# pxl-th/SLAM.jl

Hardware: AMD Instinct MI355X
Metric: frames/sec KITTI-05 stereo @1k kpts; local-BA ms/iter for 50-KF window (higher is better)
Workload: dtype f64

## Files before the change

### slam.jl_amd/csrc/common.hpp

```cpp
#pragma once
#include <hip/hip_runtime.h>
#include <cstdint>
#include <cstdio>
#include <cstring>
#include <string>
#include <vector>
#include <mutex>
#include "../../include/slamhip.h"

#define SLAM_MAX_LEVELS 8

struct slam_ctx {
    int device = 0;
    hipStream_t stream = nullptr;
    int cus = 0;
    int dev_cus = 0;
    bool arch_ok = false;
    bool xwg_ok = false;
    int pool_class = 99;
    std::string err;
    void *scratch = nullptr; size_t scratch_bytes = 0;
    void *scratch2 = nullptr; size_t scratch2_bytes = 0;
    void *pinned = nullptr; size_t pinned_bytes = 0;
    hipEvent_t wait_event = nullptr;
// ... 5 lines not shown
    std::vector<hipEvent_t> prof_pool;
    std::vector<std::string> prof_names;
    std::vector<double> prof_ms;
    std::vector<long long> prof_cnt;
};

extern "C" hipStream_t ctx_aux_stream(slam_ctx *c);
extern "C" void ctx_probe_device(slam_ctx *c);

struct ProfScope {
    slam_ctx *c; int idx;
    ProfScope(slam_ctx *ctx, const char *name);
    ~ProfScope();
};

struct LevelView {
    double *L, *Iy, *Ix, *Iyy, *Ixx, *Iyx;
    int H, W, P;
};
struct PyrView {
    LevelView lv[SLAM_MAX_LEVELS];
    int levels;
};

struct slam_pyr {
    int device = 0;
    int levels = 0;
    int H[SLAM_MAX_LEVELS], W[SLAM_MAX_LEVELS];
    int P[SLAM_MAX_LEVELS];
    int64_t off[SLAM_MAX_LEVELS + 1];
    struct Alloc { double *base = nullptr; double *ck = nullptr; double *tot = nullptr; const void **srctab = nullptr; double *xc = nullptr; int *xf = nullptr; int xseg = 0; double *rck = nullptr; int refs = 0; std::mutex graph_mu; };
    Alloc *alloc = nullptr;
    size_t zstride = 0;
    int batch_index = 0, batch_size = 1;
    bool tol_planes = false;
    bool target_only = false;
    double *planes = nullptr;
    double *tmp = nullptr;
    double *ck = nullptr;
    double *norm = nullptr;
    double norm_sigma = -1.0;
    struct Graph { int mode; double sigma; int S; size_t ckmin; int src_kind; hipGraphExec_t exec; };
    std::vector<Graph> graphs;
    bool graph_failed = false;
    PyrView view;
    double *plane(int p, int l) const { return planes + (int64_t)p * off[levels] + off[l]; }
};

struct slam_kpset {
    int device = 0, S = 0, cap = 0;
    char *base = nullptr;
    double *yx = nullptr;
    double *oyx = nullptr;
    double *syx = nullptr;
    double *xyz = nullptr;
    double *kyx = nullptr;
    uint8_t *haskf = nullptr;
    double *fyx = nullptr;
    int *fkf = nullptr;
    int *kfcount = nullptr;
    int64_t *id = nullptr;
// ... 61 lines not shown
```

### slam.jl_amd/csrc/lk.hip

```cpp
#include "common.hpp"
#include "geom_device.hpp"
#include <vector>
#include <cmath>
#include <cstdlib>

struct LKArgs {
    PyrView prev, cur;
    const double *pts, *disp0;
    int n, pyramid_levels, window, iterations;
    double eig_thr, eps, max_distance;
    double *out;
    uint8_t *status;
};

#ifdef LK_TRACE
__device__ unsigned long long g_lk_ticks[8];
#define LKT_BEGIN unsigned long long _t0 = wall_clock64()
#define LKT(k) do { const unsigned long long _t1 = wall_clock64(); if ((threadIdx.x & 63) == 0) atomicAdd(&g_lk_ticks[k], _t1 - _t0); _t0 = _t1; } while (0)
extern "C" int slam_debug_lk_ticks(unsigned long long *out)
{
    unsigned long long z[8] = {};
    if (hipMemcpyFromSymbol(out, HIP_SYMBOL(g_lk_ticks), sizeof z) != hipSuccess) return -1;
    return hipMemcpyToSymbol(HIP_SYMBOL(g_lk_ticks), z, sizeof z) == hipSuccess ? 0 : -1;
}
#else
#define LKT_BEGIN
#define LKT(k)
#endif

#define LK_OCC __attribute__((amdgpu_waves_per_eu(LK_MAXE == 9 ? 2 : 3, LK_MAXE == 9 ? 2 : 3)))
#define LK_PM 4
struct Offs { int up, down, left, right; };

__device__ __forceinline__ Offs get_offsets(int p0, int p1, double n0, double n1, int window, int H, int W)
{
    Offs o;
    const double q0 = (double)p0, q1 = (double)p1, w = (double)window;
    o.up = (int)floor(fmin(w, fmin(q0, n0) - 1));
    o.down = (int)floor(fmin(w, (double)H - fmax(q0, n0)));
    o.left = (int)floor(fmin(w, fmin(q1, n1) - 1));
    o.right = (int)floor(fmin(w, (double)W - fmax(q1, n1)));
    return o;
}

__device__ __forceinline__ double boxdiff(const double *I, int H, int y1, int y2, int x1, int x2)
{
// ... 84 lines not shown
    if (iy < 1) iy = 1;
    if (ix < 1) ix = 1;
    const double fy = r - iy, fx = c - ix;
    const double *p = img + (size_t)(iy - 1) + (size_t)(ix - 1) * P;
    const int dy = H > 1 ? 1 : 0; const size_t dx = W > 1 ? (size_t)P : 0;
    const double r0 = (1 - fx) * p[0] + fx * p[dx];
    const double r1 = (1 - fx) * p[dy] + fx * p[dy + dx];
    return (1 - fy) * r0 + fy * r1;
}

__device__ __forceinline__ bool lies_in(int H, int W, double a, double b)
{
    return 1.0 <= a && a <= (double)H && 1.0 <= b && b <= (double)W;
}

template <int LK_MAXE> struct Tmpl {
    double t0[LK_MAXE], t1[LK_MAXE], t2[LK_MAXE];
    int pq[LK_MAXE];
    int ne, kmax;
};
struct __attribute__((packed, aligned(8))) D2 { double a, b; };

template <int LK_MAXE, bool TOL>
__device__ __forceinline__ void load_template(Tmpl<LK_MAXE> &T, const LevelView &first, int p0, int p1, Offs o)
{
    const int lane = threadIdx.x & 63, pitch = first.P;
    const int P = o.up + o.down + 1, Q = o.left + o.right + 1, NE = P * Q;
    T.ne = NE; T.kmax = (NE + 63) >> 6;
    int pe, qe, sp, sq;
    if (P == 19) { pe = lane % 19; qe = lane / 19; sp = 64 % 19; sq = 64 / 19; }
    else if (P == 13) { pe = lane % 13; qe = lane / 13; sp = 64 % 13; sq = 64 / 13; }
    else if (P == 23) { pe = lane % 23; qe = lane / 23; sp = 64 % 23; sq = 64 / 23; }
    else { pe = lane % P; qe = lane / P; sp = 64 % P; sq = 64 / P; }
#pragma unroll
    for (int k = 0; k < LK_MAXE; k++) {
        const int e = lane + 64 * k;
        const bool in = e < NE;
        const int p = in ? pe : 0, q = in ? qe : 0;
        pe += sp; qe += sq;
        if (pe >= P) { pe -= P; qe++; }
        const size_t a = (size_t)(p0 - o.up + p - 1) + (size_t)(p1 - o.left + q - 1) * pitch;
        double v0 = 0.0, v1 = 0.0, v2 = 0.0;
        if (in) { v0 = first.L[a]; v1 = first.Iy[a]; v2 = first.Ix[a]; }
        T.t0[k] = in ? v0 : 0.0; T.t1[k] = in ? v1 : 0.0; T.t2[k] = in ? v2 : 0.0;
        T.pq[k] = TOL ? p + q * (2 * (LK_MAXE == 3 ? 6 : LK_MAXE == 6 ? 9 : 11) + 2 + 2 * LK_PM) : (p | (q << 16));
    }
}

template <int LK_MAXE> struct PatchGeom {
    static constexpr int WMAX = LK_MAXE == 3 ? 6 : LK_MAXE == 6 ? 9 : 11;
    static constexpr int PS = 2 * WMAX + 2 + 2 * LK_PM;
};
template <int PS>
__device__ __forceinline__ void stage_patch(double *patch, const double *img, int H, int W, int pitch, int cy, int cx, int &pry, int &prx)
{
    const int lane = threadIdx.x & 63;
    const int hy = H - PS, hx = W - PS;
    pry = cy < 0 ? 0 : (cy > hy ? (hy > 0 ? hy : 0) : cy);
    prx = cx < 0 ? 0 : (cx > hx ? (hx > 0 ? hx : 0) : cx);
    constexpr int CPC = PS / 2;
    constexpr int CPI = 64 / CPC;
    constexpr int NIT = (PS + CPI - 1) / CPI;
    const int ch = lane % CPC, c = lane / CPC;
    const double *src = img + (size_t)pry + (size_t)prx * pitch + (2 * ch + (size_t)c * pitch);
    const bool rows_ok = pry + 2 * ch < H;
#pragma unroll
    for (int i = 0; i < NIT; i++) {
        if (c < CPI && i * CPI + c < PS && rows_ok && prx + i * CPI + c < W)
            __builtin_amdgcn_global_load_lds((const __attribute__((address_space(1))) void *)(src + (size_t)(i * CPI) * pitch),
                                             (__attribute__((address_space(3))) void *)(patch + i * CPI * PS), 16, 0, 0);
    }
}

template <int LK_MAXE, bool TOL>
__device__ __forceinline__ bool lk_level(const LevelView &first, const LevelView &second, int level,
                         double pty, double ptx, double &dy, double &dx,
                         int window, int iterations, double eig_thr, double eps)
{
    const int lane = threadIdx.x & 63;
    const int H = first.H, W = first.W, pitch = first.P;
    const double iscale = __hiloint2double((1023 - (level - 1)) << 20, 0);
    const int p0 = (int)floor(pty * iscale), p1 = (int)floor(ptx * iscale);
    const double pf0 = (double)p0, pf1 = (double)p1;
    LKT_BEGIN;
    const bool cached = (2 * window + 1) * (2 * window + 1) <= 64 * LK_MAXE;
    Tmpl<LK_MAXE> T;
    constexpr int PS = PatchGeom<LK_MAXE>::PS;
    __shared__ __attribute__((aligned(16))) double lds_patch[PS * PS];
    int pry = 0, prx = 0;
    const int pmarg = (PS - (2 * window + 2)) >> 1;
    Offs o = {0, 0, 0, 0};
    double Gi[4];
    double c0 = 0.0, c1 = 0.0;
    for (int it = -1; it < iterations; it++) {
        double r0 = pf0, r1 = pf1;
        if (it >= 0) {
            const double f0 = dy + c0, f1 = dx + c1;
            r0 = pf0 + f0; r1 = pf1 + f1;
            if (!lies_in(H, W, r0, r1)) return false;
        }
        const Offs no = get_offsets(p0, p1, r0, r1, window, H, W);
        LKT(5);
        const double e0 = it < 0 ? pf0 + dy : r0, e1 = it < 0 ? pf1 + dx : r1;
        const double fr0 = floor(e0), fr1 = floor(e1);
        const int iy0 = (int)fr0, ix0 = (int)fr1;
        const bool fast = cached && iy0 - no.up >= 1 && iy0 + no.down <= H - 1 && ix0 - no.left >= 1 && ix0 + no.right <= W - 1;
        const int fy0 = iy0 - no.up - 1, fx0 = ix0 - no.left - 1;
        if (cached && (it < 0 || (fast && (fy0 < pry || iy0 + no.down > pry + PS - 1 || fx0 < prx || ix0 + no.right > prx + PS - 1))))
            stage_patch<PS>(lds_patch, second.L, H, W, pitch, iy0 - window - 1 - pmarg, ix0 - window - 1 - pmarg, pry, prx);
        if (it < 0 || no.up != o.up || no.down != o.down || no.left != o.left || no.right != o.right) {
            o = no;
            if (cached) load_template<LK_MAXE, TOL>(T, first, p0, p1, o);
            const double min_eig = spatial_gradient(first, p0, p1, o, Gi);
            LKT(1);
            if (min_eig < eig_thr) return false;
            LKT(2);
        }
        if (it < 0) continue;
        double ay = 0.0, ax = 0.0;
        if (fast) {
            asm volatile("s_waitcnt vmcnt(0)" ::: "memory");
            const double *pb = lds_patch + (fy0 - pry) + (fx0 - prx) * PS;
            constexpr int HS = (LK_MAXE + 1) / 2;
            if (TOL) {
                const double fy = r0 - fr0, fx = r1 - fr1;
#pragma unroll
                for (int h0 = 0; h0 < LK_MAXE; h0 += HS) {
                    D2 c0v[HS], c1v[HS];
#pragma unroll
                    for (int j = 0; j < HS; j++) {
                        const int k = h0 + j;
                        if (k < LK_MAXE && k < T.kmax) { const double *ptr = pb + T.pq[k]; c0v[j] = *(const D2 *)ptr; c1v[j] = *(const D2 *)(ptr + PS); }
                    }
#pragma unroll
                    for (int j = 0; j < HS; j++) {
                        const int k = h0 + j;
                        if (k < LK_MAXE && k < T.kmax) {
                            const double t0 = __builtin_fma(fx, c1v[j].a - c0v[j].a, c0v[j].a);
                            const double t1 = __builtin_fma(fx, c1v[j].b - c0v[j].b, c0v[j].b);
                            const double dI = T.t0[k] - __builtin_fma(fy, t1 - t0, t0);
                            ay = __builtin_fma(dI, T.t1[k], ay); ax = __builtin_fma(dI, T.t2[k], ax);
                        }
                    }
                }
            } else
#pragma unroll
            for (int h0 = 0; h0 < LK_MAXE; h0 += HS) {
                D2 c0v[HS], c1v[HS];
#pragma unroll
                for (int j = 0; j < HS; j++) {
                    const int k = h0 + j;
                    if (k < LK_MAXE && k < T.kmax) {
                        const double *ptr = pb + ((T.pq[k] & 0xffff) + (T.pq[k] >> 16) * PS);
                        c0v[j] = *(const D2 *)ptr; c1v[j] = *(const D2 *)(ptr + PS);
                    }
                }
#pragma unroll
                for (int j = 0; j < HS; j++) {
                    const int k = h0 + j;
                    if (k < LK_MAXE && k < T.kmax) {
                        const double dp = (double)((T.pq[k] & 0xffff) - o.up), dq = (double)((T.pq[k] >> 16) - o.left);
                        const double fy = (r0 + dp) - (fr0 + dp), fx = (r1 + dq) - (fr1 + dq);
                        const double t0 = (1 - fx) * c0v[j].a + fx * c1v[j].a;
                        const double t1 = (1 - fx) * c0v[j].b + fx * c1v[j].b;
                        const double dI = T.t0[k] - ((1 - fy) * t0 + fy * t1);
                        ay += dI * T.t1[k];
                        ax += dI * T.t2[k];
                    }
                }
            }
        } else {
            const int P = o.up + o.down + 1, Q = o.left + o.right + 1, NE = P * Q;
            for (int e = lane; e < NE; e += 64) {
                const int p = e % P, q = e / P;
                const double r = r0 + (double)(p - o.up), c = r1 + (double)(q - o.left);
                const size_t a = (size_t)(p0 - o.up + p - 1) + (size_t)(p1 - o.left + q - 1) * pitch;
                const double dI = first.L[a] - bilinear(second.L, H, W, pitch, r, c);
                ay += dI * first.Iy[a];
                ax += dI * first.Ix[a];
            }
        }
        LKT(3);
        wave_sum2(ay, ax);
        const double fl0 = TOL ? __builtin_fma(Gi[0], ay, Gi[2] * ax) : Gi[0] * ay + Gi[2] * ax, fl1 = TOL ? __builtin_fma(Gi[1], ay, Gi[3] * ax) : Gi[1] * ay + Gi[3] * ax;
        if (fabs(fl0) < eps && fabs(fl1) < eps) break;
        c0 += fl0; c1 += fl1;
        if (!lies_in(H, W, r0 + fl0, r1 + fl1)) return false;
        LKT(4);
    }
    dy += c0; dx += c1;
    if (level > 1) { dy *= 2.0; dx *= 2.0; }
    return true;
}

__device__ __forceinline__ LevelView shifted(const LevelView &v, size_t off)
{
    LevelView r = v;
    r.L += off; r.Iy += off; r.Ix += off; r.Iyy += off; r.Ixx += off; r.Iyx += off;
    return r;
}

template <int LK_MAXE, bool TOL = false>
__device__ __forceinline__ bool fb_point(const PyrView &prev, const PyrView &cur, double py, double px, double dy, double dx,
                                         int pyramid_levels, int window, int iterations, double eig_thr, double eps,
                                         double max_distance, double &ny, double &nx, size_t offP = 0, size_t offC = 0)
{
    double qy = py, qx = px, cy = dy, cx = dx;
    for (int k = 0; k <= pyramid_levels + 1; k++) {
        const bool back = k == pyramid_levels + 1;
        const int level = back ? 1 : pyramid_levels + 1 - k;
        if (back) {
            ny = py + cy; nx = px + cx;
            qy = ny; qx = nx;
// ... 333 lines not shown
```

### slam.jl_amd/csrc/pyramid.hip

```cpp
#include "common.hpp"
#include <cmath>
#include <cstdlib>
#include <mutex>
#include <tuple>
#include <utility>

#define LINE_THREADS 64

struct PlaneSet {
    double *p[4];
    const double *nrm[4];
    int coef[4];
    int fill0[4];
    const double *sq[4];
    int n;
    size_t zs;
};
#define PS_PICK(ps, f, pl) ((pl) == 0 ? (ps).f[0] : (pl) == 1 ? (ps).f[1] : (pl) == 2 ? (ps).f[2] : (ps).f[3])
__device__ __forceinline__ double *ps_plane(const PlaneSet &ps, int pl) { return PS_PICK(ps, p, pl) + (size_t)blockIdx.z * ps.zs; }
__device__ __forceinline__ const double *ps_nrm(const PlaneSet &ps, int pl) { return PS_PICK(ps, nrm, pl); }
__device__ __forceinline__ int ps_coef(const PlaneSet &ps, int pl) { return PS_PICK(ps, coef, pl); }
__device__ __forceinline__ bool ps_fill0(const PlaneSet &ps, int pl) { return PS_PICK(ps, fill0, pl) != 0; }
__device__ __forceinline__ const double *ps_sq(const PlaneSet &ps, int pl) { const double *q = PS_PICK(ps, sq, pl); return q ? q + (size_t)blockIdx.z * ps.zs : nullptr; }

// ... 106 lines not shown
    __device__ __forceinline__ bool valid() const { const int c = x0 + (int)(threadIdx.x & 63); return c >= slo && c <= shi; }
    __device__ __forceinline__ double ld_src(int i) const { return src[(size_t)i + (size_t)xown() * P]; }
    __device__ __forceinline__ double ld_dst(int i) const { return dst[(size_t)i + (size_t)xown() * P]; }
    __device__ __forceinline__ void st(int i, double v) const { if (valid()) dst[(size_t)i + (size_t)xown() * P] = v; }
    __device__ __forceinline__ void fence() const { __builtin_amdgcn_fence(__ATOMIC_RELEASE, "workgroup"); __builtin_amdgcn_fence(__ATOMIC_ACQUIRE, "workgroup"); }

    __device__ __forceinline__ void tile_load(const double *base, int rb, double t[16]) const
    {
        const int lane = threadIdx.x & 63, rp = lane & 7, cg = lane >> 3;
        const unsigned voff = (unsigned)(cg * P + 2 * rp);
#pragma unroll
        for (int r = 0; r < 8; r++) {
            const double *cb = base + ((size_t)(x0 + 8 * r) * P + rb);
            const double2 q = *(const double2 *)(cb + voff);
            t[2 * r] = q.x; t[2 * r + 1] = q.y;
        }
    }
    __device__ __forceinline__ void tile_store(int rb, const double t[16], int lo, int hi, bool partial) const
    {
        const int lane = threadIdx.x & 63, rp = lane & 7, cg = lane >> 3;
        const int row = rb + 2 * rp;
        const unsigned voff = (unsigned)(cg * P + 2 * rp);
#pragma unroll
        for (int r = 0; r < 8; r++) {
            const int col = x0 + 8 * r + cg;
            if (col >= slo && col <= shi) {
                double *q = dst + ((size_t)(x0 + 8 * r) * P + rb) + voff;
                if (!partial && nt) { const v2d v = {t[2 * r], t[2 * r + 1]}; __builtin_nontemporal_store(v, (v2d *)q); }
                else if (!partial) *(double2 *)q = make_double2(t[2 * r], t[2 * r + 1]);
                else {
// ... 360 lines not shown
    iir_rows_ck<false>(ps, H, W, P, cf, ck, rz);
}
__global__ __launch_bounds__(LINE_THREADS) void k_iir_rows_ck_odd(PlaneSet ps, int H, int W, int P, IIRPair cf, double *ck, RowResize rz)
{
    iir_rows_ck<true>(ps, H, W, P, cf, ck, rz);
}

__global__ __launch_bounds__(LINE_THREADS) void k_iir_cols_ck(PlaneSet ps, const double *src0, int H, int W, int P, IIRPair cf, double *ck)
{
    if (src0) src0 += (size_t)blockIdx.z * ps.zs;
    __shared__ __attribute__((aligned(16))) double tile[64 * COL_LS];
    const int pl = blockIdx.y, lane = threadIdx.x & 63;
    ColIO<2> io;
    const double *sqsrc = ps_sq(ps, pl);
    const bool sq = sqsrc != nullptr;
    io.dst = ps_plane(ps, pl); io.src = sq ? sqsrc : ((pl == 0 && src0) ? src0 : io.dst);
    io.H = H; io.W = W; io.P = P; io.x0 = blockIdx.x * LINE_THREADS; io.lds = tile; io.slo = 0; io.shi = W - 1; io.nt = true;
    const size_t nlines = (size_t)gridDim.z * gridDim.y * gridDim.x * LINE_THREADS;
    const size_t lineid = (((size_t)blockIdx.z * gridDim.y + pl) * gridDim.x + blockIdx.x) * LINE_THREADS + lane;
    const int n = H;
    const IIRCoef &k = ps_coef(ps, pl) == 0 ? cf.c[0] : cf.c[1];
    const bool fill0 = ps_fill0(ps, pl);
    const double a1 = k.a1, a2 = k.a2, a3 = k.a3, scale = k.scale;
    auto in = [&](double v) { return sq ? v * v : v; };
    const double x0 = in(io.ld_src(0));
    const double iminus = fill0 ? 0.0 : x0, iplus = fill0 ? 0.0 : in(io.ld_src(n - 1));
    const double uminus = iminus / k.inv1masum;
    const double o0 = ((x0 + a1 * uminus) + a2 * uminus) + a3 * uminus;
    const double o1 = ((in(io.ld_src(1)) + a1 * o0) + a2 * uminus) + a3 * uminus;
    const double o2 = ((in(io.ld_src(2)) + a1 * o1) + a2 * o0) + a3 * uminus;
    double w3 = o0, w2 = o1, w1 = o2;
    double raw[32], x[32];
    {
        const int NT = ((n - 1) >> 4) + 1;
        io.tile_load(io.src, 0, raw);
        for (int t = 0; t < NT; t++) {
            const int rb = t << 4;
            io.lds_put_tile(raw); io.template lds_get_col<+1>(x);
            if (sq) {
#pragma unroll
                for (int e = 0; e < 16; e++) x[e] = x[e] * x[e];
            }
            if (t + 1 < NT) io.tile_load(io.src, rb + 16, raw);
            if ((t & 1) == 0 && t >= 2) { double *c = ck + ((size_t)(t >> 1) * 3) * nlines + lineid; c[0] = w1; c[nlines] = w2; c[2 * nlines] = w3; }
            if (rb >= 3 && rb + 15 <= n - 1) {
#pragma unroll
                for (int e = 0; e < 16; e++) { const double tt = ((x[e] + a1 * w1) + a2 * w2) + a3 * w3; w3 = w2; w2 = w1; w1 = tt; }
            } else {
#pragma unroll
                for (int e = 0; e < 16; e++) { const int row = rb + e; if (row >= 3 && row <= n - 1) { const double tt = ((x[e] + a1 * w1) + a2 * w2) + a3 * w3; w3 = w2; w2 = w1; w1 = tt; } }
            }
        }
    }
    const double uplus = iplus / k.inv1masum, vplus = uplus / k.inv1mbsum;
    const double d0 = w1 - uplus, d1 = w2 - uplus, d2 = w3 - uplus;
    const double vr0 = ((k.M[0] * d0 + k.M[1] * d1) + k.M[2] * d2) + vplus;
    const double vr1 = ((k.M[3] * d0 + k.M[4] * d1) + k.M[5] * d2) + vplus;
    const double vr2 = ((k.M[6] * d0 + k.M[7] * d1) + k.M[8] * d2) + vplus;
    const double vA = vr0;
    const double vB = ((w2 + a1 * vA) + a2 * vr1) + a3 * vr2;
    const double vC = ((w3 + a1 * vB) + a2 * vA) + a3 * vr1;
    double v1 = vC, v2 = vB, v3 = vA;
    io.fence();
    const int NBk = ((n - 4) >> 5) + 1;
    const int ntile = P >> 4;
    auto load_block = [&](int b) {
        io.tile_load(io.src, b << 5, raw);
        if (2 * b + 1 < ntile) io.tile_load(io.src, (b << 5) + 16, raw + 16);
    };
    if (n - 4 >= 3) load_block(NBk - 1);
    io.st(n - 1, vA * scale); io.st(n - 2, vB * scale); io.st(n - 3, vC * scale);
    for (int b = NBk - 1; b >= 0 && n - 4 >= 3; b--) {
        const int rb = b << 5, lo = rb > 3 ? rb : 3, hi = rb + 31 < n - 4 ? rb + 31 : n - 4;
        const bool two = 2 * b + 1 < ntile;
        io.lds_put_tile(raw); io.template lds_get_col<+1>(x);
        if (two) { io.lds_put_tile(raw + 16); io.template lds_get_col<+1>(x + 16); }
        if (sq) {
#pragma unroll
            for (int e = 0; e < 32; e++) x[e] = x[e] * x[e];
        }
        if (b > 0) load_block(b - 1);
        double f1, f2, f3;
        if (b > 0) { const double *c = ck + ((size_t)b * 3) * nlines + lineid; f1 = c[0]; f2 = c[nlines]; f3 = c[2 * nlines]; }
// ... 16 lines not shown
            io.template lds_put_col<+1>(x + 16); io.lds_get_tile(u);
            io.tile_store(rb + 16, u, lo, hi, !(lo <= rb + 16 && hi >= rb + 31));
        }
    }
    {
        double tt = ((o2 + a1 * v1) + a2 * v2) + a3 * v3; v3 = v2; v2 = v1; v1 = tt; io.st(2, tt * scale);
        tt = ((o1 + a1 * v1) + a2 * v2) + a3 * v3; v3 = v2; v2 = v1; v1 = tt; io.st(1, tt * scale);
        tt = ((o0 + a1 * v1) + a2 * v2) + a3 * v3; io.st(0, tt * scale);
    }
}

#define CF4_COLS 62
struct ColsFusedArgs {
    const double *L;
    double *T;
    double *Iy, *Ix, *Qyy, *Qxx, *Qyx;
    int H, W, P; size_t zs;
    int src_kind; const void *const *srctab;
    double *tot; int tot_stride;
    int dec;
};

template <bool TOL>
__device__ __forceinline__ double iir3(double x, double a1, double w1, double a2, double w2, double a3, double w3)
{
    if (TOL) return __builtin_fma(a1, w1, __builtin_fma(a2, w2, __builtin_fma(a3, w3, x)));
    return ((x + a1 * w1) + a2 * w2) + a3 * w3;
}
template <bool TOL>
__device__ __forceinline__ void scharr_pair(double a, double b, double c, double &d, double &s)
{
// ... 89 lines not shown
__device__ __forceinline__ void cols_fused_wave(const ColsFusedArgs &A, const IIRCoef &k, double *ck, double *LB, double *IYB, double *IXB, double *QB, const double *lut)
{
    const int lane = threadIdx.x & 63, rp = lane & 7, cg = lane >> 3;
    const int H = A.H, W = A.W, P = A.P, n = H;
    const int own0 = CF4_COLS * (int)blockIdx.x;
    const int xl = own0 > 0 ? own0 - 1 : 0;
    const size_t z = (size_t)blockIdx.z * A.zs;
    const bool active = ROLE != 0 || A.T != nullptr;
    const int nroles = A.T != nullptr ? 4 : 3;
    double *stage = ROLE == 0 ? LB : ROLE == 1 ? IYB : ROLE == 2 ? IXB : QB;
    ColIO<2> io;
    io.src = A.L + z;
    io.dst = (ROLE == 0 ? A.T : ROLE == 1 ? A.Qyy : ROLE == 2 ? A.Qxx : A.Qyx) + z;
    io.H = H; io.W = W; io.P = P; io.x0 = xl; io.lds = stage;
    io.slo = own0; io.shi = own0 + CF4_COLS - 1 < W - 1 ? own0 + CF4_COLS - 1 : W - 1; io.nt = true;
    ColIO<2> iog = io;
    iog.dst = (ROLE == 1 ? A.Iy : A.Ix) + z;
    const int col = xl + lane;
    const bool edgeL = col == 0, edgeR = col == W - 1;
    const size_t nlines = (size_t)gridDim.z * nroles * gridDim.x * LINE_THREADS;
    const size_t lineid = (((size_t)blockIdx.z * nroles + (ROLE - (4 - nroles))) * gridDim.x + blockIdx.x) * LINE_THREADS + lane;
    const double a1 = k.a1, a2 = k.a2, a3 = k.a3, scale = k.scale;
    const int w = ROLE;
    const int skind = A.src_kind;
    typedef const __attribute__((address_space(1))) double *gsrc_f64;
    typedef const __attribute__((address_space(1))) unsigned char *gsrc_u8;
    typedef const __attribute__((address_space(3))) double *lds_f64;
    const void *simg = skind ? A.srctab[blockIdx.z] : nullptr;
    const gsrc_f64 simg_d = (gsrc_f64)simg; const gsrc_u8 simg_b = (gsrc_u8)simg; const lds_f64 lutl = (lds_f64)lut;
    auto src_at = [&](int row, int colx) -> double {
        return skind == 1 ? simg_d[(size_t)row + (size_t)colx * H] : lutl[simg_b[(size_t)row + (size_t)colx * H]];
    };
// ... 158 lines not shown
        lds_barrier();  
        if (active) read_inputs();
        if (ROLE == 0 && skind) {
            ColIO<2> iol = io; iol.dst = const_cast<double *>(A.L) + z;
            const int ghi = H - 1;
#pragma unroll
            for (int t = 0; t < 2; t++) {
                if (t == 0 || (two && rb + 16 <= ghi)) {
#pragma unroll
                    for (int r = 0; r < 8; r++) { const double2 q = *(const double2 *)(LB + (8 * r + cg) * CF4_LS + 2 + 16 * t + 2 * rp); u[2 * r] = q.x; u[2 * r + 1] = q.y; }
                    iol.tile_store(rb + 16 * t, u, rb + 16 * t, ghi, rb + 16 * t + 15 > ghi);
                }
            }
        }
        if (ROLE == 1 || ROLE == 2) {
            const double *blk = ROLE == 1 ? IYB : IXB;
            const int ghi = H - 1;
            get_tile(blk, 0, u); iog.tile_store(rb, u, rb, ghi, rb + 15 > ghi);
            if (two && rb + 16 <= ghi) { get_tile(blk, 1, u); iog.tile_store(rb + 16, u, rb + 16, ghi, rb + 31 > ghi); }
        }
        lds_barrier();
        double f1 = f1n, f2 = f2n, f3 = f3n;
        if (b > 0) { prefetch(b - 1); if (active) load_ck(b - 1); }
        if (!active || (lo > hi && !dec)) continue;
        if (lo > hi) {}
        else if (lo == rb && hi == rb + 31) {
#pragma unroll
            for (int e = 0; e < 32; e++) { const double tt = iir3<TOL>(x[e], a1, f1, a2, f2, a3, f3); f3 = f2; f2 = f1; f1 = tt; x[e] = tt; }
#pragma unroll
            for (int e = 31; e >= 0; e--) { const double tt = iir3<TOL>(x[e], a1, v1, a2, v2, a3, v3); v3 = v2; v2 = v1; v1 = tt;
                                            if (SFX) { x[e] = sfx; sfx = __builtin_fma(tt, scale, sfx); } else x[e] = tt * scale; }
        } else {
#pragma unroll
            for (int e = 0; e < 32; e++) { const int row = rb + e; if (row >= lo && row <= hi) { const double tt = iir3<TOL>(x[e], a1, f1, a2, f2, a3, f3); f3 = f2; f2 = f1; f1 = tt; x[e] = tt; } }
// ... 836 lines not shown
    ColTerm t; t.d = 0.0; t.s = 0.0;
    if (border == 0) xx = xx < 0 ? 0 : (xx >= W ? W - 1 : xx);
    else if (xx < 0 || xx >= W) return t;
    const double *c0 = L + (size_t)xx * P;
    double a, b, c;
    b = c0[y];
    if (border == 0) { a = c0[y > 0 ? y - 1 : 0]; c = c0[y + 1 < H ? y + 1 : H - 1]; }
    else { a = y > 0 ? c0[y - 1] : 0.0; c = y + 1 < H ? c0[y + 1] : 0.0; }
    t.d += a * dk[0]; t.d += b * dk[1]; t.d += c * dk[2];
    t.s += a * sk[0]; t.s += b * sk[1]; t.s += c * sk[2];
    return t;
}
template <int XC>
__global__ __launch_bounds__(64) void k_scharr_products(LevelView v, int border, size_t zs, int squares)
{
    { const size_t z = (size_t)blockIdx.z * zs; v.L += z; v.Iy += z; v.Ix += z; v.Iyy += z; v.Ixx += z; v.Iyx += z; }
    const int H = v.H, W = v.W, P = v.P;
    const int y = blockIdx.x * 64 + threadIdx.x;
    if (y >= H) return;
    const int xs = blockIdx.y * XC, xe = min(W, xs + XC);
    const double dk[3] = {-1.0 / 2, 0.0 / 2, 1.0 / 2}, sk[3] = {3.0 / 16, 10.0 / 16, 3.0 / 16};
    ColTerm t0 = scharr_col(v.L, H, W, P, y, xs - 1, border), t1 = scharr_col(v.L, H, W, P, y, xs, border);
    for (int x = xs; x < xe; x++) {
        const ColTerm t2 = scharr_col(v.L, H, W, P, y, x + 1, border);
        double iy = 0.0, ix = 0.0;
        iy += t0.d * sk[0]; iy += t1.d * sk[1]; iy += t2.d * sk[2];
        ix += t0.s * dk[0]; ix += t1.s * dk[1]; ix += t2.s * dk[2];
        const size_t i = (size_t)y + (size_t)x * P;
        v.Iy[i] = iy; v.Ix[i] = ix;
        if (squares) { v.Iyy[i] = iy * iy; v.Ixx[i] = ix * ix; }
        v.Iyx[i] = iy * ix;
        t0 = t1; t1 = t2;
    }
}

__global__ __launch_bounds__(256) void k_resize(double *dst, int Hd, int Wd, int Pd, const double *src, int Hs, int Ws, int Ps, size_t zs)
{
    dst += (size_t)blockIdx.z * zs; src += (size_t)blockIdx.z * zs;
    const size_t i = (size_t)blockIdx.x * 256 + threadIdx.x;
    if (i >= (size_t)Hd * Wd) return;
    const int y = (int)(i % Hd) + 1, x = (int)(i / Hd) + 1;
    const double sy = (double)Hs / (double)Hd, sx = (double)Ws / (double)Wd;
    const double oy = 1 - 0.5 - sy * (1 - 0.5), ox = 1 - 0.5 - sx * (1 - 0.5);
    double r = sy * y + oy, c = sx * x + ox;
// ... 19 lines not shown
}

#define BATCH_MAX 128
struct ImgPtrs { const double *p[BATCH_MAX]; };
__global__ __launch_bounds__(256) void k_gather_images(ImgPtrs src, double *dst, int H, int W, int P, size_t zs)
{
    const size_t i = (size_t)blockIdx.x * 256 + threadIdx.x;
    if (i < (size_t)H * W) dst[(size_t)blockIdx.z * zs + i % H + (i / H) * P] = src.p[blockIdx.z][i];
}
struct ImgPtrsU8 { const unsigned char *p[BATCH_MAX]; };
__global__ __launch_bounds__(256) void k_gather_images_u8(ImgPtrsU8 src, double *dst, int H, int W, int P, size_t zs)
{
    const size_t i = (size_t)blockIdx.x * 256 + threadIdx.x;
    if (i < (size_t)H * W) dst[(size_t)blockIdx.z * zs + i % H + (i / H) * P] = (double)src.p[blockIdx.z][i] / 255.0;
}
__global__ __launch_bounds__(256) void k_unpitch(double *dst, const double *src, int H, int W, int P)
{
    const size_t i = (size_t)blockIdx.x * 256 + threadIdx.x;
    if (i < (size_t)H * W) dst[i] = src[i % H + (i / H) * P];
}

__global__ __launch_bounds__(256) void k_fill(double *p, size_t n, double v)
{
    const size_t i = (size_t)blockIdx.x * 256 + threadIdx.x;
    if (i < n) p[i] = v;
}

struct PyrKnobs {
    static bool set(const char *name) { return getenv(name) != nullptr; }
    static int num(const char *name, int dflt) { const char *e = getenv(name); return e ? atoi(e) : dflt; }
    const int tol_batch_min_s = num("SLAMHIP_TOL_BATCH_MIN_S", 4);
    const int chunk_mb = num("SLAMHIP_PYR_CHUNK_MB", 0);
    const int scharr_xc1 = num("SLAMHIP_SCHARR_XC1", 2);
    const int rt_dbg = num("SLAMHIP_RT_DBG", 0);
// ... 10 lines not shown
}
static inline dim3 lines_grid(int nlines, int nplanes, int S = 1) { return dim3((nlines + LINE_THREADS - 1) / LINE_THREADS, nplanes, S); }
static inline int rz_odd_bands(int H) { return (H - 1 + RZ_ODD_ROWS - 1) / RZ_ODD_ROWS; }
static inline bool rz_odd_ok(const slam_pyr *p, int l)
{
    if (knobs().no_rows_resize_odd || l + 1 >= p->levels) return false;
    const int H = p->H[l], W = p->W[l], Wd = p->W[l + 1];
    return H >= 3 && 2 * p->H[l + 1] - 1 == H && (W == 2 * Wd || W == 2 * Wd - 1) && rz_odd_bands(H) <= 4 * ((p->H[0] + LINE_THREADS - 1) / LINE_THREADS);
}

static void make_view(slam_pyr *p)
{
    p->view.levels = p->levels;
    for (int l = 0; l < p->levels; l++) {
        LevelView &v = p->view.lv[l];
        v.L = p->plane(0, l); v.Iy = p->plane(1, l); v.Ix = p->plane(2, l);
        v.Iyy = p->plane(3, l); v.Ixx = p->plane(4, l); v.Iyx = p->plane(5, l);
        v.H = p->H[l]; v.W = p->W[l]; v.P = p->P[l];
    }
}

static int build_norm(slam_ctx *ctx, slam_pyr *p, double sigma)
{
    if (p->norm && p->norm_sigma == sigma) return SLAM_OK;
    if (!p->norm) HIP_TRY(ctx, hipMalloc((void **)&p->norm, ((size_t)p->off[p->levels] + (size_t)64 * p->P[0]) * 8));
    IIRPair cf; cf.c[0] = slam_iir_coef(sigma); cf.c[1] = cf.c[0];
    for (int l = 0; l + 1 < p->levels; l++) {
        double *N = p->norm + p->off[l];
        size_t n = (size_t)p->P[l] * p->W[l];
        hipLaunchKernelGGL(k_fill, dim3((n + 255) / 256), dim3(256), 0, ctx->stream, N, n, 1.0);
        PlaneSet ps = {}; ps.p[0] = N; ps.coef[0] = 0; ps.fill0[0] = 1; ps.n = 1;
// ... 154 lines not shown
    return r;
}
struct LevelIO {
    int H, W, P; LevelView v; double *T;
    RowResize next;
    const double *norm; double *tot;
    size_t zs; int z0;
    int src_kind; const void *const *srctab;
};
static LevelIO level_io(const slam_pyr *p, int l, int z0, int Sall, int src_kind)
{
    LevelIO io = {};
    const size_t zo = (size_t)z0 * p->zstride;
    io.H = p->H[l]; io.W = p->W[l]; io.P = p->P[l]; io.zs = p->zstride; io.z0 = z0;
    io.v = p->view.lv[l];
    io.v.L += zo; io.v.Iy += zo; io.v.Ix += zo; io.v.Iyy += zo; io.v.Ixx += zo; io.v.Iyx += zo;
    io.T = p->tmp + p->off[l] + zo;
    if (l + 1 < p->levels) io.next = RowResize{p->view.lv[l + 1].L + zo, p->H[l + 1], p->W[l + 1], p->P[l + 1]};
    io.norm = p->norm ? p->norm + p->off[l] : nullptr;
    size_t toff = (size_t)3 * z0 * io.W;
    for (int q = 0; q < l; q++) toff += (size_t)3 * Sall * p->W[q];
    io.tot = p->alloc->tot ? p->alloc->tot + toff : nullptr;
    io.src_kind = l == 0 ? src_kind : 0; io.srctab = (const void *const *)p->alloc->srctab + z0;
    return io;
}
static PlaneSet plane_slice(const PlaneSet &ps, int first, int n, bool with_sq = true)
{
    PlaneSet s = {};
    for (int q = 0, f = first; q < n; q++, f++) { s.p[q] = ps.p[f]; s.nrm[q] = ps.nrm[f]; s.coef[q] = ps.coef[f]; s.fill0[q] = ps.fill0[f]; s.sq[q] = with_sq ? ps.sq[f] : nullptr; }
    s.n = n; s.zs = ps.zs;
    return s;
}
static PlaneSet level_planes(const LevelRoute &r, const LevelIO &io)
{
    PlaneSet ps = {}; int np = 0;
    if (r.has_next) { ps.p[np] = io.T; ps.coef[np] = 0; ps.fill0[np] = r.zero_border; ps.nrm[np] = r.zero_border ? io.norm : nullptr; np++; }
    ps.p[np] = io.v.Iyy; ps.coef[np] = 1; ps.sq[np] = r.fuse_sq ? io.v.Iy : nullptr; np++;
    ps.p[np] = io.v.Ixx; ps.coef[np] = 1; ps.sq[np] = r.fuse_sq ? io.v.Ix : nullptr; np++;
    ps.p[np] = io.v.Iyx; ps.coef[np] = 1; np++;
    ps.n = np; ps.zs = io.zs;
    return ps;
}
static PlaneSet cum_planes(const LevelIO &io) { PlaneSet pc = {}; pc.p[0] = io.v.Iyy; pc.p[1] = io.v.Ixx; pc.p[2] = io.v.Iyx; pc.n = 3; pc.zs = io.zs; return pc; }
static RowResize row_resize(const LevelRoute &r, const LevelIO &io) { return (r.resize == RZ_EVEN || r.resize == RZ_ODD) ? io.next : RowResize{}; }
static RowsTolArgs rows_tol_args(const LevelRoute &r, const LevelIO &io, bool layer, int product_kind)
{
    RowsTolArgs ra = {}; int n = 0;
    if (layer) { ra.p[n] = io.T; ra.coef[n] = 0; ra.kind[n] = 0; ra.rz = row_resize(r, io); n++; }
    ra.nq0 = n;
    if (product_kind) for (double *q : {io.v.Iyy, io.v.Ixx, io.v.Iyx}) { ra.p[n] = q; ra.coef[n] = 1; ra.kind[n] = product_kind; n++; }
    ra.n = n; ra.zs = io.zs;
    return ra;
}
// ... 8 lines not shown
    if (r.scharr_xc == 1) SCH_GO(1); else if (r.scharr_xc == 2) SCH_GO(2); else if (r.scharr_xc == 4) SCH_GO(4); else if (r.scharr_xc == 8) SCH_GO(8);
    else if (r.scharr_xc) SCH_GO(SCH_XC);
#undef SCH_GO
}
static void launch_cols(BuildSink &B, const LevelRoute &r, int lane, const PlaneSet &ps, const double *src0, int S, const LevelIO &io, const IIRPair &cf, double *ck)
{
    const dim3 g = lines_grid(io.W, ps.n, S);
    if (r.cols == COLS_CK) B.launch(k_iir_cols_ck, g, dim3(LINE_THREADS), 0, lane, ps, src0, io.H, io.W, io.P, cf, ck);
    else if (r.line_c == 3) B.launch(k_iir_cols<3>, g, dim3(LINE_THREADS), 0, lane, ps, src0, io.H, io.W, io.P, cf);
    else B.launch(k_iir_cols<2>, g, dim3(LINE_THREADS), 0, lane, ps, src0, io.H, io.W, io.P, cf);
}
static void launch_cols_fused(BuildSink &B, const LevelRoute &r, const LevelIO &io, int S, const IIRPair &cf, double *ck)
{
    const bool tol = r.rows == ROWS_TOL;
    ColsFusedArgs ca;
    ca.L = io.v.L; ca.T = r.has_next ? io.T : nullptr; ca.Iy = io.v.Iy; ca.Ix = io.v.Ix; ca.Qyy = io.v.Iyy; ca.Qxx = io.v.Ixx; ca.Qyx = io.v.Iyx;
    ca.H = io.H; ca.W = io.W; ca.P = io.P; ca.zs = io.zs;
    ca.src_kind = io.src_kind; ca.srctab = io.srctab;
    ca.tot = tol ? io.tot : nullptr; ca.tot_stride = io.W; ca.dec = r.dec ? 1 : 0;
    const dim3 g((io.W + CF4_COLS - 1) / CF4_COLS, 1, S);
    if (tol && r.dec) B.launch(k_cols_fused<true, true>, g, dim3(256), 0, LN_MAIN, ca, cf, ck);
    else if (tol) B.launch(k_cols_fused<true, false>, g, dim3(256), 0, LN_MAIN, ca, cf, ck);
    else B.launch(k_cols_fused<false, false>, g, dim3(256), 0, LN_MAIN, ca, cf, ck);
}
static void launch_rows(BuildSink &B, const LevelRoute &r, int lane, const PlaneSet &ps, int S, const LevelIO &io, const IIRPair &cf, double *ck)
{
    const RowResize rz = row_resize(r, io);
    if (r.rows == ROWS_CK && r.resize == RZ_ODD) B.launch(k_iir_rows_ck_odd, dim3(rz_odd_bands(io.H), 1, S), dim3(LINE_THREADS), 0, lane, ps, io.H, io.W, io.P, cf, ck, rz);
    else if (r.rows == ROWS_CK) B.launch(k_iir_rows_ck, lines_grid(io.H, ps.n, S), dim3(LINE_THREADS), 0, lane, ps, io.H, io.W, io.P, cf, ck, rz);
    else B.launch(k_iir_rows, lines_grid(io.H, ps.n, S), dim3(LINE_THREADS), 0, lane, ps, io.H, io.W, io.P, cf);
}
// ... 370 lines not shown
    if (W) *W = p->W[level];
    return SLAM_OK;
}

int slam_pyr_levels(const slam_pyr *p) { return p ? p->levels : SLAM_ERR_ARG; }

int slam_pyr_download(slam_ctx *ctx, const slam_pyr *p, int plane, int level, double *out)
{
    ARG_TRY(ctx, ctx != nullptr && p != nullptr && out != nullptr);
    ARG_TRY(ctx, plane >= 0 && plane < 6 && level >= 0 && level < p->levels);
    HIP_TRY(ctx, hipSetDevice(ctx->device));
    const size_t n = (size_t)p->H[level] * p->W[level];
    void *stage;
    int rc = slam_scratch2(ctx, n * 8, &stage);
    if (rc) return rc;
    hipLaunchKernelGGL(k_unpitch, dim3((n + 255) / 256), dim3(256), 0, ctx->stream, (double *)stage, (const double *)p->plane(plane, level), p->H[level], p->W[level], p->P[level]);
    HIP_TRY(ctx, hipMemcpyAsync(out, stage, n * 8, hipMemcpyDeviceToHost, ctx->stream));
    HIP_TRY(ctx, slam_stream_wait(ctx->stream));
    return SLAM_OK;
}

}
```

Before: 23920.

## Interleave Iy/Ix gradient planes into a GradPair array for paired loads

Replaces the separate Iy and Ix pyramid planes with one interleaved 16-byte GradPair array. LK template loads and the slow path then fetch both gradients in a single vector load, and the Scharr and fused-column kernels write them together with nontemporal stores. The IIR squared-input path and the download path are adapted to the stride-2 layout. It also splits the LDS patch size into separate row and column margins (both still 4) and adds debug counters. The change carries a risk of uncoalesced stride-2 reads in the IIR column loader.

```diff
diff --git a/slam.jl_amd/csrc/common.hpp b/slam.jl_amd/csrc/common.hpp
--- a/slam.jl_amd/csrc/common.hpp
+++ b/slam.jl_amd/csrc/common.hpp
@@ -43,9 +43,11 @@
     ~ProfScope();
 };
 
+struct __attribute__((aligned(16))) GradPair { double iy, ix; };
 struct LevelView {
-    double *L, *Iy, *Ix, *Iyy, *Ixx, *Iyx;
+    double *L; GradPair *G; double *Iyy, *Ixx, *Iyx;
     int H, W, P;
+    __host__ __device__ void shift(size_t doubles) { L += doubles; G = (GradPair *)((double *)G + doubles); Iyy += doubles; Ixx += doubles; Iyx += doubles; }
 };
 struct PyrView {
     LevelView lv[SLAM_MAX_LEVELS];
@@ -74,6 +76,7 @@
     bool graph_failed = false;
     PyrView view;
     double *plane(int p, int l) const { return planes + (int64_t)p * off[levels] + off[l]; }
+    GradPair *grad(int l) const { return (GradPair *)(planes + off[levels] + 2 * off[l]); }
 };
 
 struct slam_kpset {
diff --git a/slam.jl_amd/csrc/lk.hip b/slam.jl_amd/csrc/lk.hip
--- a/slam.jl_amd/csrc/lk.hip
+++ b/slam.jl_amd/csrc/lk.hip
@@ -17,6 +17,7 @@
 __device__ unsigned long long g_lk_ticks[8];
 #define LKT_BEGIN unsigned long long _t0 = wall_clock64()
 #define LKT(k) do { const unsigned long long _t1 = wall_clock64(); if ((threadIdx.x & 63) == 0) atomicAdd(&g_lk_ticks[k], _t1 - _t0); _t0 = _t1; } while (0)
+#define LKC(k) do { if ((threadIdx.x & 63) == 0) atomicAdd(&g_lk_ticks[k], 1ull); } while (0)
 extern "C" int slam_debug_lk_ticks(unsigned long long *out)
 {
     unsigned long long z[8] = {};
@@ -26,10 +27,12 @@
 #else
 #define LKT_BEGIN
 #define LKT(k)
+#define LKC(k)
 #endif
 
 #define LK_OCC __attribute__((amdgpu_waves_per_eu(LK_MAXE == 9 ? 2 : 3, LK_MAXE == 9 ? 2 : 3)))
-#define LK_PM 4
+#define LK_PMR 4
+#define LK_PMC 4
 struct Offs { int up, down, left, right; };
 
 __device__ __forceinline__ Offs get_offsets(int p0, int p1, double n0, double n1, int window, int H, int W)
@@ -144,6 +147,7 @@
     return 1.0 <= a && a <= (double)H && 1.0 <= b && b <= (double)W;
 }
 
+template <int LK_MAXE> struct PatchGeom;
 template <int LK_MAXE> struct Tmpl {
     double t0[LK_MAXE], t1[LK_MAXE], t2[LK_MAXE];
     int pq[LK_MAXE];
@@ -171,34 +175,35 @@
         if (pe >= P) { pe -= P; qe++; }
         const size_t a = (size_t)(p0 - o.up + p - 1) + (size_t)(p1 - o.left + q - 1) * pitch;
         double v0 = 0.0, v1 = 0.0, v2 = 0.0;
-        if (in) { v0 = first.L[a]; v1 = first.Iy[a]; v2 = first.Ix[a]; }
+        if (in) { v0 = first.L[a]; const GradPair g = first.G[a]; v1 = g.iy; v2 = g.ix; }
         T.t0[k] = in ? v0 : 0.0; T.t1[k] = in ? v1 : 0.0; T.t2[k] = in ? v2 : 0.0;
-        T.pq[k] = TOL ? p + q * (2 * (LK_MAXE == 3 ? 6 : LK_MAXE == 6 ? 9 : 11) + 2 + 2 * LK_PM) : (p | (q << 16));
+        T.pq[k] = TOL ? p + q * PatchGeom<LK_MAXE>::PSR : (p | (q << 16));
     }
 }
 
 template <int LK_MAXE> struct PatchGeom {
     static constexpr int WMAX = LK_MAXE == 3 ? 6 : LK_MAXE == 6 ? 9 : 11;
-    static constexpr int PS = 2 * WMAX + 2 + 2 * LK_PM;
+    static constexpr int PSR = 2 * WMAX + 2 + 2 * LK_PMR;
+    static constexpr int PSC = 2 * WMAX + 2 + 2 * LK_PMC;
 };
-template <int PS>
+template <int PSR, int PSC>
 __device__ __forceinline__ void stage_patch(double *patch, const double *img, int H, int W, int pitch, int cy, int cx, int &pry, int &prx)
 {
     const int lane = threadIdx.x & 63;
-    const int hy = H - PS, hx = W - PS;
+    const int hy = H - PSR, hx = W - PSC;
     pry = cy < 0 ? 0 : (cy > hy ? (hy > 0 ? hy : 0) : cy);
     prx = cx < 0 ? 0 : (cx > hx ? (hx > 0 ? hx : 0) : cx);
-    constexpr int CPC = PS / 2;
+    constexpr int CPC = PSR / 2;
     constexpr int CPI = 64 / CPC;
-    constexpr int NIT = (PS + CPI - 1) / CPI;
+    constexpr int NIT = (PSC + CPI - 1) / CPI;
     const int ch = lane % CPC, c = lane / CPC;
     const double *src = img + (size_t)pry + (size_t)prx * pitch + (2 * ch + (size_t)c * pitch);
     const bool rows_ok = pry + 2 * ch < H;
 #pragma unroll
     for (int i = 0; i < NIT; i++) {
-        if (c < CPI && i * CPI + c < PS && rows_ok && prx + i * CPI + c < W)
+        if (c < CPI && i * CPI + c < PSC && rows_ok && prx + i * CPI + c < W)
             __builtin_amdgcn_global_load_lds((const __attribute__((address_space(1))) void *)(src + (size_t)(i * CPI) * pitch),
-                                             (__attribute__((address_space(3))) void *)(patch + i * CPI * PS), 16, 0, 0);
+                                             (__attribute__((address_space(3))) void *)(patch + i * CPI * PSR), 16, 0, 0);
     }
 }
 
@@ -215,10 +220,10 @@
     LKT_BEGIN;
     const bool cached = (2 * window + 1) * (2 * window + 1) <= 64 * LK_MAXE;
     Tmpl<LK_MAXE> T;
-    constexpr int PS = PatchGeom<LK_MAXE>::PS;
-    __shared__ __attribute__((aligned(16))) double lds_patch[PS * PS];
+    constexpr int PSR = PatchGeom<LK_MAXE>::PSR, PSC = PatchGeom<LK_MAXE>::PSC;
+    __shared__ __attribute__((aligned(16))) double lds_patch[PSR * PSC];
     int pry = 0, prx = 0;
-    const int pmarg = (PS - (2 * window + 2)) >> 1;
+    const int pmr = (PSR - (2 * window + 2)) >> 1, pmc = (PSC - (2 * window + 2)) >> 1;
     Offs o = {0, 0, 0, 0};
     double Gi[4];
     double c0 = 0.0, c1 = 0.0;
@@ -236,8 +241,8 @@
         const int iy0 = (int)fr0, ix0 = (int)fr1;
         const bool fast = cached && iy0 - no.up >= 1 && iy0 + no.down <= H - 1 && ix0 - no.left >= 1 && ix0 + no.right <= W - 1;
         const int fy0 = iy0 - no.up - 1, fx0 = ix0 - no.left - 1;
-        if (cached && (it < 0 || (fast && (fy0 < pry || iy0 + no.down > pry + PS - 1 || fx0 < prx || ix0 + no.right > prx + PS - 1))))
-            stage_patch<PS>(lds_patch, second.L, H, W, pitch, iy0 - window - 1 - pmarg, ix0 - window - 1 - pmarg, pry, prx);
+        if (cached && (it < 0 || (fast && (fy0 < pry || iy0 + no.down > pry + PSR - 1 || fx0 < prx || ix0 + no.right > prx + PSC - 1))))
+            { stage_patch<PSR, PSC>(lds_patch, second.L, H, W, pitch, iy0 - window - 1 - pmr, ix0 - window - 1 - pmc, pry, prx); LKC(6); if (it < 0) LKC(7); }
         if (it < 0 || no.up != o.up || no.down != o.down || no.left != o.left || no.right != o.right) {
             o = no;
             if (cached) load_template<LK_MAXE, TOL>(T, first, p0, p1, o);
@@ -250,7 +255,7 @@
         double ay = 0.0, ax = 0.0;
         if (fast) {
             asm volatile("s_waitcnt vmcnt(0)" ::: "memory");
-            const double *pb = lds_patch + (fy0 - pry) + (fx0 - prx) * PS;
+            const double *pb = lds_patch + (fy0 - pry) + (fx0 - prx) * PSR;
             constexpr int HS = (LK_MAXE + 1) / 2;
             if (TOL) {
                 const double fy = r0 - fr0, fx = r1 - fr1;
@@ -260,7 +265,7 @@
 #pragma unroll
                     for (int j = 0; j < HS; j++) {
                         const int k = h0 + j;
-                        if (k < LK_MAXE && k < T.kmax) { const double *ptr = pb + T.pq[k]; c0v[j] = *(const D2 *)ptr; c1v[j] = *(const D2 *)(ptr + PS); }
+                        if (k < LK_MAXE && k < T.kmax) { const double *ptr = pb + T.pq[k]; c0v[j] = *(const D2 *)ptr; c1v[j] = *(const D2 *)(ptr + PSR); }
                     }
 #pragma unroll
                     for (int j = 0; j < HS; j++) {
@@ -281,8 +286,8 @@
                 for (int j = 0; j < HS; j++) {
                     const int k = h0 + j;
                     if (k < LK_MAXE && k < T.kmax) {
-                        const double *ptr = pb + ((T.pq[k] & 0xffff) + (T.pq[k] >> 16) * PS);
-                        c0v[j] = *(const D2 *)ptr; c1v[j] = *(const D2 *)(ptr + PS);
+                        const double *ptr = pb + ((T.pq[k] & 0xffff) + (T.pq[k] >> 16) * PSR);
+                        c0v[j] = *(const D2 *)ptr; c1v[j] = *(const D2 *)(ptr + PSR);
                     }
                 }
 #pragma unroll
@@ -306,8 +311,9 @@
                 const double r = r0 + (double)(p - o.up), c = r1 + (double)(q - o.left);
                 const size_t a = (size_t)(p0 - o.up + p - 1) + (size_t)(p1 - o.left + q - 1) * pitch;
                 const double dI = first.L[a] - bilinear(second.L, H, W, pitch, r, c);
-                ay += dI * first.Iy[a];
-                ax += dI * first.Ix[a];
+                const GradPair g = first.G[a];
+                ay += dI * g.iy;
+                ax += dI * g.ix;
             }
         }
         LKT(3);
@@ -326,7 +332,7 @@
 __device__ __forceinline__ LevelView shifted(const LevelView &v, size_t off)
 {
     LevelView r = v;
-    r.L += off; r.Iy += off; r.Ix += off; r.Iyy += off; r.Ixx += off; r.Iyx += off;
+    r.shift(off);
     return r;
 }
 
diff --git a/slam.jl_amd/csrc/pyramid.hip b/slam.jl_amd/csrc/pyramid.hip
--- a/slam.jl_amd/csrc/pyramid.hip
+++ b/slam.jl_amd/csrc/pyramid.hip
@@ -144,6 +144,19 @@
             const double *cb = base + ((size_t)(x0 + 8 * r) * P + rb);
             const double2 q = *(const double2 *)(cb + voff);
             t[2 * r] = q.x; t[2 * r + 1] = q.y;
+        }
+    }
+    __device__ __forceinline__ void tile_load_pair(const double *base, int rb, double t[16]) const
+    {
+        const int lane = threadIdx.x & 63, rp = lane & 7, cg = lane >> 3;
+        const unsigned voff = (unsigned)(2 * (cg * P + 2 * rp));
+#pragma unroll
+        for (int r = 0; r < 8; r++) {
+            t[2 * r] = 0.0; t[2 * r + 1] = 0.0;
+            if (x0 + 8 * r < W) {
+                const double *cb = base + 2 * ((size_t)(x0 + 8 * r) * P + rb);
+                t[2 * r] = cb[voff]; t[2 * r + 1] = cb[voff + 2];
+            }
         }
     }
     __device__ __forceinline__ void tile_store(int rb, const double t[16], int lo, int hi, bool partial) const
@@ -534,7 +547,7 @@
     ColIO<2> io;
     const double *sqsrc = ps_sq(ps, pl);
     const bool sq = sqsrc != nullptr;
-    io.dst = ps_plane(ps, pl); io.src = sq ? sqsrc : ((pl == 0 && src0) ? src0 : io.dst);
+    io.dst = ps_plane(ps, pl); io.src = (pl == 0 && src0) ? src0 : io.dst;
     io.H = H; io.W = W; io.P = P; io.x0 = blockIdx.x * LINE_THREADS; io.lds = tile; io.slo = 0; io.shi = W - 1; io.nt = true;
     const size_t nlines = (size_t)gridDim.z * gridDim.y * gridDim.x * LINE_THREADS;
     const size_t lineid = (((size_t)blockIdx.z * gridDim.y + pl) * gridDim.x + blockIdx.x) * LINE_THREADS + lane;
@@ -542,18 +555,19 @@
     const IIRCoef &k = ps_coef(ps, pl) == 0 ? cf.c[0] : cf.c[1];
     const bool fill0 = ps_fill0(ps, pl);
     const double a1 = k.a1, a2 = k.a2, a3 = k.a3, scale = k.scale;
-    auto in = [&](double v) { return sq ? v * v : v; };
-    const double x0 = in(io.ld_src(0));
-    const double iminus = fill0 ? 0.0 : x0, iplus = fill0 ? 0.0 : in(io.ld_src(n - 1));
+    auto in = [&](int i) { if (!sq) return io.ld_src(i); const double v = sqsrc[2 * ((size_t)i + (size_t)io.xown() * P)]; return v * v; };
+    auto tile_in = [&](int rb, double *t) { if (sq) io.tile_load_pair(sqsrc, rb, t); else io.tile_load(io.src, rb, t); };
+    const double x0 = in(0);
+    const double iminus = fill0 ? 0.0 : x0, iplus = fill0 ? 0.0 : in(n - 1);
     const double uminus = iminus / k.inv1masum;
     const double o0 = ((x0 + a1 * uminus) + a2 * uminus) + a3 * uminus;
-    const double o1 = ((in(io.ld_src(1)) + a1 * o0) + a2 * uminus) + a3 * uminus;
-    const double o2 = ((in(io.ld_src(2)) + a1 * o1) + a2 * o0) + a3 * uminus;
+    const double o1 = ((in(1) + a1 * o0) + a2 * uminus) + a3 * uminus;
+    const double o2 = ((in(2) + a1 * o1) + a2 * o0) + a3 * uminus;
     double w3 = o0, w2 = o1, w1 = o2;
     double raw[32], x[32];
     {
         const int NT = ((n - 1) >> 4) + 1;
-        io.tile_load(io.src, 0, raw);
+        tile_in(0, raw);
         for (int t = 0; t < NT; t++) {
             const int rb = t << 4;
             io.lds_put_tile(raw); io.template lds_get_col<+1>(x);
@@ -561,7 +575,7 @@
 #pragma unroll
                 for (int e = 0; e < 16; e++) x[e] = x[e] * x[e];
             }
-            if (t + 1 < NT) io.tile_load(io.src, rb + 16, raw);
+            if (t + 1 < NT) tile_in(rb + 16, raw);
             if ((t & 1) == 0 && t >= 2) { double *c = ck + ((size_t)(t >> 1) * 3) * nlines + lineid; c[0] = w1; c[nlines] = w2; c[2 * nlines] = w3; }
             if (rb >= 3 && rb + 15 <= n - 1) {
 #pragma unroll
@@ -585,8 +599,8 @@
     const int NBk = ((n - 4) >> 5) + 1;
     const int ntile = P >> 4;
     auto load_block = [&](int b) {
-        io.tile_load(io.src, b << 5, raw);
-        if (2 * b + 1 < ntile) io.tile_load(io.src, (b << 5) + 16, raw + 16);
+        tile_in(b << 5, raw);
+        if (2 * b + 1 < ntile) tile_in((b << 5) + 16, raw + 16);
     };
     if (n - 4 >= 3) load_block(NBk - 1);
     io.st(n - 1, vA * scale); io.st(n - 2, vB * scale); io.st(n - 3, vC * scale);
@@ -633,7 +647,7 @@
 struct ColsFusedArgs {
     const double *L;
     double *T;
-    double *Iy, *Ix, *Qyy, *Qxx, *Qyx;
+    GradPair *G; double *Qyy, *Qxx, *Qyx;
     int H, W, P; size_t zs;
     int src_kind; const void *const *srctab;
     double *tot; int tot_stride;
@@ -753,8 +767,7 @@
     io.dst = (ROLE == 0 ? A.T : ROLE == 1 ? A.Qyy : ROLE == 2 ? A.Qxx : A.Qyx) + z;
     io.H = H; io.W = W; io.P = P; io.x0 = xl; io.lds = stage;
     io.slo = own0; io.shi = own0 + CF4_COLS - 1 < W - 1 ? own0 + CF4_COLS - 1 : W - 1; io.nt = true;
-    ColIO<2> iog = io;
-    iog.dst = (ROLE == 1 ? A.Iy : A.Ix) + z;
+    double *const gdst = (double *)A.G + z;
     const int col = xl + lane;
     const bool edgeL = col == 0, edgeR = col == W - 1;
     const size_t nlines = (size_t)gridDim.z * nroles * gridDim.x * LINE_THREADS;
@@ -943,10 +956,15 @@
             }
         }
         if (ROLE == 1 || ROLE == 2) {
-            const double *blk = ROLE == 1 ? IYB : IXB;
-            const int ghi = H - 1;
-            get_tile(blk, 0, u); iog.tile_store(rb, u, rb, ghi, rb + 15 > ghi);
-            if (two && rb + 16 <= ghi) { get_tile(blk, 1, u); iog.tile_store(rb + 16, u, rb + 16, ghi, rb + 31 > ghi); }
+            const int r16 = lane & 15, rr = 16 * (ROLE - 1) + r16, row = rb + rr;
+            const double *qy = IYB + (8 * (lane >> 4)) * CF4_GS + rr, *qx = IXB + (8 * (lane >> 4)) * CF4_GS + rr;
+            double *g = gdst + 2 * ((size_t)(xl + 8 * (lane >> 4)) * P + row);
+#pragma unroll
+            for (int r = 0; r < 16; r++) {
+                const int cl = (r & 7) + 32 * (r >> 3), cx = xl + 8 * (lane >> 4) + cl;
+                const v2d v = {qy[cl * CF4_GS], qx[cl * CF4_GS]};
+                if (row < H && cx >= io.slo && cx <= io.shi) __builtin_nontemporal_store(v, (v2d *)(g + 2 * (size_t)cl * P));
+            }
         }
         lds_barrier();
         double f1 = f1n, f2 = f2n, f3 = f3n;
@@ -1813,7 +1831,7 @@
 template <int XC>
 __global__ __launch_bounds__(64) void k_scharr_products(LevelView v, int border, size_t zs, int squares)
 {
-    { const size_t z = (size_t)blockIdx.z * zs; v.L += z; v.Iy += z; v.Ix += z; v.Iyy += z; v.Ixx += z; v.Iyx += z; }
+    v.shift((size_t)blockIdx.z * zs);
     const int H = v.H, W = v.W, P = v.P;
     const int y = blockIdx.x * 64 + threadIdx.x;
     if (y >= H) return;
@@ -1826,7 +1844,7 @@
         iy += t0.d * sk[0]; iy += t1.d * sk[1]; iy += t2.d * sk[2];
         ix += t0.s * dk[0]; ix += t1.s * dk[1]; ix += t2.s * dk[2];
         const size_t i = (size_t)y + (size_t)x * P;
-        v.Iy[i] = iy; v.Ix[i] = ix;
+        v.G[i] = GradPair{iy, ix};
         if (squares) { v.Iyy[i] = iy * iy; v.Ixx[i] = ix * ix; }
         v.Iyx[i] = iy * ix;
         t0 = t1; t1 = t2;
@@ -1876,10 +1894,10 @@
     const size_t i = (size_t)blockIdx.x * 256 + threadIdx.x;
     if (i < (size_t)H * W) dst[(size_t)blockIdx.z * zs + i % H + (i / H) * P] = (double)src.p[blockIdx.z][i] / 255.0;
 }
-__global__ __launch_bounds__(256) void k_unpitch(double *dst, const double *src, int H, int W, int P)
+__global__ __launch_bounds__(256) void k_unpitch(double *dst, const double *src, int H, int W, int P, int es)
 {
     const size_t i = (size_t)blockIdx.x * 256 + threadIdx.x;
-    if (i < (size_t)H * W) dst[i] = src[i % H + (i / H) * P];
+    if (i < (size_t)H * W) dst[i] = src[(i % H) * es + (i / H) * P];
 }
 
 __global__ __launch_bounds__(256) void k_fill(double *p, size_t n, double v)
@@ -1920,7 +1938,7 @@
     p->view.levels = p->levels;
     for (int l = 0; l < p->levels; l++) {
         LevelView &v = p->view.lv[l];
-        v.L = p->plane(0, l); v.Iy = p->plane(1, l); v.Ix = p->plane(2, l);
+        v.L = p->plane(0, l); v.G = p->grad(l);
         v.Iyy = p->plane(3, l); v.Ixx = p->plane(4, l); v.Iyx = p->plane(5, l);
         v.H = p->H[l]; v.W = p->W[l]; v.P = p->P[l];
     }
@@ -2105,7 +2123,7 @@
     const size_t zo = (size_t)z0 * p->zstride;
     io.H = p->H[l]; io.W = p->W[l]; io.P = p->P[l]; io.zs = p->zstride; io.z0 = z0;
     io.v = p->view.lv[l];
-    io.v.L += zo; io.v.Iy += zo; io.v.Ix += zo; io.v.Iyy += zo; io.v.Ixx += zo; io.v.Iyx += zo;
+    io.v.shift(zo);
     io.T = p->tmp + p->off[l] + zo;
     if (l + 1 < p->levels) io.next = RowResize{p->view.lv[l + 1].L + zo, p->H[l + 1], p->W[l + 1], p->P[l + 1]};
     io.norm = p->norm ? p->norm + p->off[l] : nullptr;
@@ -2126,8 +2144,8 @@
 {
     PlaneSet ps = {}; int np = 0;
     if (r.has_next) { ps.p[np] = io.T; ps.coef[np] = 0; ps.fill0[np] = r.zero_border; ps.nrm[np] = r.zero_border ? io.norm : nullptr; np++; }
-    ps.p[np] = io.v.Iyy; ps.coef[np] = 1; ps.sq[np] = r.fuse_sq ? io.v.Iy : nullptr; np++;
-    ps.p[np] = io.v.Ixx; ps.coef[np] = 1; ps.sq[np] = r.fuse_sq ? io.v.Ix : nullptr; np++;
+    ps.p[np] = io.v.Iyy; ps.coef[np] = 1; ps.sq[np] = r.fuse_sq ? &io.v.G->iy : nullptr; np++;
+    ps.p[np] = io.v.Ixx; ps.coef[np] = 1; ps.sq[np] = r.fuse_sq ? &io.v.G->ix : nullptr; np++;
     ps.p[np] = io.v.Iyx; ps.coef[np] = 1; np++;
     ps.n = np; ps.zs = io.zs;
     return ps;
@@ -2166,7 +2184,7 @@
 {
     const bool tol = r.rows == ROWS_TOL;
     ColsFusedArgs ca;
-    ca.L = io.v.L; ca.T = r.has_next ? io.T : nullptr; ca.Iy = io.v.Iy; ca.Ix = io.v.Ix; ca.Qyy = io.v.Iyy; ca.Qxx = io.v.Ixx; ca.Qyx = io.v.Iyx;
+    ca.L = io.v.L; ca.T = r.has_next ? io.T : nullptr; ca.G = io.v.G; ca.Qyy = io.v.Iyy; ca.Qxx = io.v.Ixx; ca.Qyx = io.v.Iyx;
     ca.H = io.H; ca.W = io.W; ca.P = io.P; ca.zs = io.zs;
     ca.src_kind = io.src_kind; ca.srctab = io.srctab;
     ca.tot = tol ? io.tot : nullptr; ca.tot_stride = io.W; ca.dec = r.dec ? 1 : 0;
@@ -2567,7 +2585,9 @@
     void *stage;
     int rc = slam_scratch2(ctx, n * 8, &stage);
     if (rc) return rc;
-    hipLaunchKernelGGL(k_unpitch, dim3((n + 255) / 256), dim3(256), 0, ctx->stream, (double *)stage, (const double *)p->plane(plane, level), p->H[level], p->W[level], p->P[level]);
+    const bool grad = plane == 1 || plane == 2;
+    const double *src = grad ? (plane == 1 ? &p->grad(level)->iy : &p->grad(level)->ix) : p->plane(plane, level);
+    hipLaunchKernelGGL(k_unpitch, dim3((n + 255) / 256), dim3(256), 0, ctx->stream, (double *)stage, src, p->H[level], p->W[level], (grad ? 2 : 1) * p->P[level], grad ? 2 : 1);
     HIP_TRY(ctx, hipMemcpyAsync(out, stage, n * 8, hipMemcpyDeviceToHost, ctx->stream));
     HIP_TRY(ctx, slam_stream_wait(ctx->stream));
     return SLAM_OK;
```

After: 24100, median of 6. Within noise of the previous version (+0.8%).
